# foxcroftjn/polars-strsim

Measured on AMD Instinct MI355X. Metric: M string-pairs/s, levenshtein, 100 M rows (+ achieved HBM GB/s in roofline), higher is better.
Workload: dtype u8/u32 bit-parallel, f64 epilogue

## Files before the change

### polars-strsim_amd/csrc/strsim_capi.cpp

```cpp
#include <hip/hip_runtime.h>
#include <algorithm>

#include <cstdarg>
#include <cstdio>
#include <cstdlib>
#include <cstring>
#include <memory>
#include <new>
#include <string>

#include "strsim_amd.h"
#include "strsim_internal.h"
#include "strsim_kernels.h"
#define STRSIM_OSA_NO_KERNELS
#include "strsim_osa.h"
#include "strsim_distance.h"
#include "strsim_indel.h"
#include "strsim_partial.h"
#include "strsim_token.h"
#include "strsim_nearest.h"

namespace strsim {

static thread_local std::string g_last_error;
// ... 324 lines not shown
    if (const char *env = getenv("STRSIM_LEV_WAVES_PER_CU")) {
        const int v = atoi(env);
        if (v >= 1 && v <= 256) c->lev_waves_per_cu = v;
    }
    c->no_literal_path = getenv("STRSIM_NO_LITERAL_PATH") != nullptr;
    if (const char *env = getenv("STRSIM_WIDE_WG_PER_CU")) {
        const int v = atoi(env);
        if (v >= 1 && v <= 4096) c->wide_cap_per_cu = v;
    }
    if (const char *env = getenv("STRSIM_HUGE_WAVES_PER_CU")) {
        const int v = atoi(env);
        if (v >= 1 && v <= 32) c->huge_waves_per_cu = v;
    }
    if (const char *env = getenv("STRSIM_HOST_DIRECT_ROWS")) c->host_direct_rows = (uint64_t)strtoull(env, nullptr, 10);
    if (const char *env = getenv("STRSIM_FAULT_RETIRE_AT")) c->fault_retire_at = (uint64_t)strtoull(env, nullptr, 10);
    if (hip_stream) {
        c->stream = (hipStream_t)hip_stream;
    } else {
        e = hipStreamCreateWithFlags(&c->stream, hipStreamNonBlocking);
        if (e != hipSuccess) { delete c; return hip_fail(e, "hipStreamCreateWithFlags"); }
        c->own_stream = true;
    }
    e = hipMalloc((void **)&c->status, sizeof(DevStatus) * strsim_ctx::RING);
    if (e == hipSuccess) e = hipMalloc((void **)&c->sched, sizeof(uint32_t) * 4 * strsim_ctx::RING);
    if (e == hipSuccess) e = hipMemsetAsync(c->sched, 0, sizeof(uint32_t) * 4 * strsim_ctx::RING, c->stream);
    if (e == hipSuccess)
        e = hipHostMalloc((void **)&c->status_host, sizeof(DevStatus) * strsim_ctx::RING, hipHostMallocDefault);
    if (e != hipSuccess) { strsim_ctx_destroy(c); return hip_fail(e, "status allocation"); }
    memset(c->status_host, 0, sizeof(DevStatus) * strsim_ctx::RING);
    e = hipHostGetDevicePointer((void **)&c->status_host_dev, c->status_host, 0);
    if (e != hipSuccess) { strsim_ctx_destroy(c); return hip_fail(e, "hipHostGetDevicePointer"); }
    {
        static double q[QTAB_N * QTAB_N];
        for (int a = 0; a < QTAB_N; ++a)
            for (int b = 0; b < QTAB_N; ++b) q[a * QTAB_N + b] = b ? (double)a / (double)b : 0.0;
        e = hipMalloc((void **)&c->qtab, sizeof(q));
        if (e == hipSuccess) e = hipMemcpy(c->qtab, q, sizeof(q), hipMemcpyHostToDevice);
        if (e != hipSuccess) { strsim_ctx_destroy(c); return hip_fail(e, "quotient table"); }
    }
    *out_ctx = c;
    return STRSIM_OK;
}

void strsim_ctx_destroy(strsim_ctx_t *c)
{
    if (!c) return;
    (void)hipSetDevice(c->device);
    if (c->stream) (void)hipStreamSynchronize(c->stream);
// ... 410 lines not shown
    }
    if (two_pass_measure(measure)) return pairs_osa(c, slot, measure, a_off, a_val, a_rows, b_off, b_val, b_rows, outs[0], n);
    if (measure == STRSIM_TOKEN_SORT_RATIO || measure == STRSIM_TOKEN_SET_RATIO)
        return pairs_token(c, slot, measure, a_off, a_val, a_rows, b_off, b_val, b_rows, outs[0], n);
    const uint64_t nchunks = (n + 63) >> 6;
    bool defer = !eager && !c->expect_slow && !c->stream_ordered;
    int mb = strsim_ctx::SHARED_MASKBUF;
    if (defer) {
        defer = false;
        for (int b = 0; b < strsim_ctx::SHARED_MASKBUF; ++b)
            if (c->maskbuf_owner[b] < 0) { mb = b; defer = true; break; }
    }
    rc = c->slowmask[mb].reserve(2 * nchunks * sizeof(unsigned long long) + nchunks * sizeof(uint32_t));
    if (rc) return rc;
    unsigned long long *const mask = c->slowmask[mb].as<unsigned long long>();
    slot_begin(c, slot);
    c->status_host[slot].lane_left = LANE_LEFT_UNKNOWN;

    LaunchArgs la;
    la.offA = a_off; la.valA = a_val; la.rowsA = a_rows;
    la.offB = b_off; la.valB = b_val; la.rowsB = b_rows;
    la.out = outs[0]; la.n = n;
    la.slowmask = mask; la.status = c->status + slot; la.stream = c->stream;
    la.sched = c->sched + 4 * slot;
    la.publish_host = nullptr;
    la.publish_ticket = 0u;
    la.worklist = reinterpret_cast<uint32_t *>(mask + 2 * nchunks);
    la.qtab = c->qtab;
    la.stage_grid = c->num_cu * c->stage_wg_per_cu;
    la.no_literal_path = c->no_literal_path;
    la.long_rows = c->long_rows;
    la.wide_grid = c->num_cu * 3;
    la.wide_grid_cap = c->num_cu * c->wide_cap_per_cu;
    la.wave_grid = c->num_cu * 16;
    la.wave_grid_lev = c->num_cu * c->lev_waves_per_cu;
    {
        const size_t waves = (size_t)std::max(la.wave_grid, la.wave_grid_lev);
        rc = c->lev_ws.reserve(waves * LEV_WS_WORDS * sizeof(uint32_t));
        if (rc) return rc;
        la.lev_ws = c->lev_ws.as<uint32_t>();
    }
    la.ev_lane0 = la.ev_lane1 = la.ev_wave1 = nullptr;
    if (c->timing) {
        for (int i = 0; i < 3; ++i)
            if (!c->ev[slot][i]) HIP_TRY(hipEventCreateWithFlags(&c->ev[slot][i], hipEventDisableSystemFence));
        la.ev_lane0 = c->ev[slot][0]; la.ev_lane1 = c->ev[slot][1]; la.ev_wave1 = c->ev[slot][2];
    }
// ... 657 lines not shown
```

### polars-strsim_amd/csrc/strsim_kernels.h

```cpp
#pragma once
#include <hip/hip_runtime.h>
#include <stdint.h>

#include "strsim_lane_core.h"

namespace strsim {

constexpr int WAVE_CAP = 1024;

#ifndef STRSIM_LEV_JOBS
#define STRSIM_LEV_JOBS 16
#endif
constexpr int LEV_JOBS = STRSIM_LEV_JOBS;
#ifndef STRSIM_LEV_BYTES_ROWS
#define STRSIM_LEV_BYTES_ROWS 64
#endif
constexpr int LEV_BYTES_ROWS = STRSIM_LEV_BYTES_ROWS;
#ifndef STRSIM_LEV_POOL
#define STRSIM_LEV_POOL 384
#endif
constexpr int LEV_POOL = STRSIM_LEV_POOL;
constexpr int TXT_PAD = 48;
constexpr int ARENA0_BYTES = 8192;
constexpr int ARENA1_BYTES = 12288;
constexpr int PAT1_BYTES = 64 * 32 * 2;
constexpr int LEV_WS_WORDS = 3 * (WAVE_CAP + 64) + (ARENA0_BYTES + ARENA1_BYTES + PAT1_BYTES) / 4;

#define HUGE_WS_WORDS(cap) (6u * ((uint64_t)(cap) + 64u) + 64u)

struct DevStatus {
    unsigned int wave_rows;
    unsigned int huge_rows;
    unsigned int max_len;
    unsigned int lane_left;
    unsigned int list_count[5];
    unsigned int list_rows[5];
    unsigned int next_entry[5];
    unsigned int pad1[12];
    unsigned int ticket;
};
static_assert(sizeof(DevStatus) == 128, "DevStatus is 128 bytes");

struct LaunchArgs {
    const uint32_t *offA; const uint8_t *valA; uint64_t rowsA;
    const uint32_t *offB; const uint8_t *valB; uint64_t rowsB;
    double *out; uint64_t n;
    unsigned long long *slowmask;
    uint32_t *worklist;
    const double *qtab;
    DevStatus *status;
    uint32_t *sched;
    DevStatus *publish_host;
    uint32_t publish_ticket;
    hipStream_t stream;
    int wide_grid, wave_grid;
    bool no_literal_path;
    bool long_rows;
    int stage_grid;
    int wide_grid_cap;
    int wave_grid_lev;
    uint32_t *lev_ws;
    hipEvent_t ev_lane0, ev_lane1, ev_wave1;
};

// ... 85 lines not shown
```

### polars-strsim_amd/csrc/strsim_lane_stage.h

```cpp
#pragma once

#ifndef STRSIM_STAGE_ROWS
#define STRSIM_STAGE_ROWS 512
#endif
#ifndef STRSIM_STAGE_CAP
#define STRSIM_STAGE_CAP 10240
#endif
#ifndef STRSIM_STAGE_CAP_LONG
#define STRSIM_STAGE_CAP_LONG 15104
#endif
#ifndef STRSIM_STAGE_CAP_LUT
#define STRSIM_STAGE_CAP_LUT 8960
#endif
#ifndef STRSIM_STAGE_WAVES_PER_EU
#define STRSIM_STAGE_WAVES_PER_EU 5
#endif
#ifndef STRSIM_STAGE_BUCKET_SHIFT
#define STRSIM_STAGE_BUCKET_SHIFT 1
#endif

#ifndef STRSIM_STAGE_LUT
#define STRSIM_STAGE_LUT 0x26
#endif
#ifndef STRSIM_JARO_KEEP_EQ_FILLS
#define STRSIM_JARO_KEEP_EQ_FILLS 1
#endif
#ifndef STRSIM_STAGE_LONG_TEXT_MAX
#define STRSIM_STAGE_LONG_TEXT_MAX 32
#endif
#ifndef STRSIM_STAGE_RANGE_MAX
#define STRSIM_STAGE_RANGE_MAX 64
#endif
#ifndef STRSIM_STAGE_RANGE_DIV
#define STRSIM_STAGE_RANGE_DIV 4
#endif
#ifndef STRSIM_STAGE_RANGE_MIN_BLOCKS
#define STRSIM_STAGE_RANGE_MIN_BLOCKS 2
#endif

#if defined(STRSIM_LAB) && defined(STRSIM_STAGE_STAMPS)
__device__ unsigned long long g_stage_stamps[16384][16];
#define STAGE_STAMP(cat) do { __builtin_amdgcn_sched_barrier(0); const unsigned long long t_ = __builtin_amdgcn_s_memtime(); \
                              __builtin_amdgcn_sched_barrier(0); st_acc[cat] += t_ - st_last; st_last = t_; } while (0)
#else
#define STAGE_STAMP(cat) do { } while (0)
#endif

#ifndef STRSIM_STAGE_THREADS
#define STRSIM_STAGE_THREADS 256
#endif
constexpr int STAGE_BLOCK = STRSIM_STAGE_THREADS;
constexpr int STAGE_WAVES = STAGE_BLOCK / 64;
constexpr int STAGE_ROWS = STRSIM_STAGE_ROWS;
constexpr int STAGE_RPT = STAGE_ROWS / STAGE_BLOCK;
constexpr int STAGE_NR = STAGE_ROWS / 64;
constexpr int STAGE_RPW = STAGE_NR / STAGE_WAVES;
template <int MEASURE> constexpr bool stage_uses_lut() { return ((STRSIM_STAGE_LUT >> MEASURE) & 1) != 0; }

template <bool TABLES, bool LONG = false> struct StageGeom {
    static_assert(!(TABLES && LONG), "the long-row geometry has no match-mask tables");
// ... 228 lines not shown
    constexpr bool LEV = MEASURE == LEVENSHTEIN;
    constexpr bool ALL = MEASURE == ALL_MEASURES;
    constexpr int B = STAGE_ROWS, RPT = STAGE_RPT, NBK = STAGE_NBK;
    constexpr int STAGE_CAP = StageGeom<LUT, LONG>::CAP, STAGE_COL = StageGeom<LUT, LONG>::COL;
    constexpr int STAGE_DMA_ITERS = StageGeom<LUT, LONG>::DMA_ITERS;
    constexpr uint32_t COLB = STAGE_COL, LIT = 2u * STAGE_COL;
    static_assert(!LUT || (B <= 128 * STAGE_WAVES && LUT_WAVE_BYTES == 3072), "descriptor slices: 128 rows behind each wave's tables");
    __shared__ __attribute__((aligned(4096))) uint8_t s_lut[LUT ? 4096 * STAGE_WAVES : 16];
    __shared__ uint2 s_desc_own[LUT ? 1 : B];
    __shared__ __attribute__((aligned(4096))) uint8_t s_bytes[2 * STAGE_COL + 64 + 16];
    auto desc_at = [&](uint32_t p) -> uint2 * {
        if (LUT) return reinterpret_cast<uint2 *>(s_lut + ((p >> 7) << 12) + LUT_WAVE_BYTES + ((p & 127u) << 3));
        return s_desc_own + p;
    };
    __shared__ __attribute__((aligned(16))) uint32_t s_off[2][B + 4];
    __shared__ uint32_t s_cnt[32];
    __shared__ uint32_t s_left;
    __shared__ uint32_t s_sched[2];
    __shared__ uint16_t s_code[LEV ? B : 1];
    __shared__ uint32_t s_word[(!LEV && !ALL) ? B : 1];
    __shared__ double s_val[ALL ? B : 1];

    const uint32_t tid = threadIdx.x, lane = lane_id(), wv = tid >> 6;
    if (blockIdx.x == 0u && tid < (uint32_t)(sizeof(DevStatus) / sizeof(uint32_t))) reinterpret_cast<uint32_t *>(status)[tid] = 0u;
    if (tid < 32u) s_cnt[tid] = 0u;
    if (tid == 0u) s_left = 0u;
#pragma unroll
    for (int q = 0; q < RPT; ++q) {
        const uint32_t i = (uint32_t)q * STAGE_BLOCK + tid;
        if (LEV) s_code[i] = 0xFFFFu;
        else if (ALL) reinterpret_cast<unsigned long long *>(&s_val[i])[0] = ~0ull;
        else s_word[i] = 0xFFFFFFFFu;
    }

    const uint32_t totalA = load_invariant(offA + rowsA), totalB = load_invariant(offB + rowsB);
#if STRSIM_BOUNDS_ON
    const uint32_t firstA = load_invariant(offA), firstB = load_invariant(offB);
#endif
    const bool bcastA = rowsA == 1, bcastB = rowsB == 1;
    const uint32_t litA0 = bcastA ? load_invariant(offA) : 0u, litB0 = bcastB ? load_invariant(offB) : 0u;
    const uint32_t litAlen = bcastA ? totalA - litA0 : 0u, litBlen = bcastB ? totalB - litB0 : 0u;
    if (wv == 0u) {
        auto literal_window = [&](const uint8_t *val, uint32_t at, uint32_t total, uint32_t len, uint32_t *dst) {
            uint32_t w[8];
            load_window32(val, at, total, w);
            const uint32_t rep = (w[0] & 0xFFu) * 0x01010101u;
#pragma unroll
            for (int q = 0; q < 8; ++q) {
                const uint32_t v = len > 4u * q ? (len - 4u * q < 4u ? len - 4u * q : 4u) : 0u;
                const uint32_t keep = v >= 4u ? 0xFFFFFFFFu : ((1u << (8u * v)) - 1u);
                dst[q] = (w[q] & keep) | (rep & ~keep);
            }
        };
        if (bcastA) literal_window(valA, litA0, totalA, litAlen, reinterpret_cast<uint32_t *>(s_bytes + LIT));
        if (bcastB) literal_window(valB, litB0, totalB, litBlen, reinterpret_cast<uint32_t *>(s_bytes + LIT + 32u));
    }
    const uint64_t nchunks = (n + 63u) >> 6;
    const uint32_t nchunks32 = (uint32_t)nchunks;
    auto grab = [&](uint32_t seen, uint32_t &lo, uint32_t &sz) {
        const uint32_t left = nchunks32 > seen ? nchunks32 - seen : 0u;
        uint32_t want = (uint32_t)STRSIM_STAGE_RANGE_MAX;
        if (left < (uint32_t)(STRSIM_STAGE_RANGE_MAX * STRSIM_STAGE_RANGE_DIV) * gridDim.x) want = left / ((uint32_t)STRSIM_STAGE_RANGE_DIV * gridDim.x);
        sz = want < (uint32_t)(STRSIM_STAGE_RANGE_MIN_BLOCKS * (B / 64)) ? (uint32_t)(STRSIM_STAGE_RANGE_MIN_BLOCKS * (B / 64)) : want;
        lo = __hip_atomic_fetch_add(&sched[0], sz, __ATOMIC_RELAXED, __HIP_MEMORY_SCOPE_AGENT);
    };
    uint32_t grab_lo = 0u, grab_sz = 0u;
    if (tid == 0u) {
        grab(0u, grab_lo, grab_sz);
        s_sched[0] = grab_lo;
        s_sched[1] = grab_sz;
    }
    lds_barrier();
    uint64_t row_end;
    uint64_t row0;
    {
        const uint64_t lo = uniform(s_sched[0]), hi = lo + uniform(s_sched[1]);
        row0 = lo * 64u < n ? lo * 64u : n;
        row_end = hi * 64u < n ? hi * 64u : n;
    }
    lds_barrier();
    if (tid == 0u) grab(grab_lo, grab_lo, grab_sz);
    bool grab_pending = true;

    EqLut lut;
    lut.lane4 = lane * 4u;
    lut.krep = ((STRSIM_LDS_ADDR(&s_lut[0]) >> 8) + 16u * wv) * 0x01010101u;
    const uint32_t ldsOffA = STRSIM_LDS_ADDR(&s_off[0][0]), ldsOffB = STRSIM_LDS_ADDR(&s_off[1][0]);
    const uint32_t ldsBytes = STRSIM_LDS_ADDR(&s_bytes[0]);
    const uint32_t wvu = uniform(wv);
    const uint32_t tid4 = tid * 4u, tid16 = tid * 16u;
    auto dma_offsets = [&](uint64_t row) {
        const uint32_t cnt = (uint32_t)(row_end - row < (uint64_t)B ? row_end - row : (uint64_t)B);
        const uint32_t *const pa = offA + row, *const pb = offB + row;
#pragma unroll
        for (int it = 0; it < RPT; ++it) {
            if (tid + (uint32_t)it * STAGE_BLOCK <= cnt) {
                if (!bcastA) STRSIM_CHECK_INDEX(K_STAGE, 1, row, row + (uint64_t)it * STAGE_BLOCK + tid, rowsA + 1u);
                if (!bcastB) STRSIM_CHECK_INDEX(K_STAGE, 2, row, row + (uint64_t)it * STAGE_BLOCK + tid, rowsB + 1u);
                STRSIM_CHECK_INDEX(K_STAGE, 3, row, (uint32_t)it * STAGE_BLOCK + tid, B + 4);
                if (!bcastA) lds_dma_b32(pa + it * STAGE_BLOCK, tid4, ldsOffA + 4u * ((uint32_t)it * STAGE_BLOCK + wvu * 64u));
                if (!bcastB) lds_dma_b32(pb + it * STAGE_BLOCK, tid4, ldsOffB + 4u * ((uint32_t)it * STAGE_BLOCK + wvu * 64u));
            }
        }
        if (tid == 0u && cnt == (uint32_t)B) {
            if (!bcastA) STRSIM_CHECK_INDEX(K_STAGE, 4, row, row + (uint64_t)B, rowsA + 1u);
            if (!bcastB) STRSIM_CHECK_INDEX(K_STAGE, 5, row, row + (uint64_t)B, rowsB + 1u);
            if (!bcastA) lds_dma_b32(pa + B, tid4, ldsOffA + 4u * (uint32_t)B);
            if (!bcastB) lds_dma_b32(pb + B, tid4, ldsOffB + 4u * (uint32_t)B);
        }
    };

    uint64_t prev_row0 = 0;
    uint32_t prev_rows = 0;
    if (row0 < row_end) dma_offsets(row0);
    asm volatile("s_waitcnt vmcnt(0)" ::: "memory");
    lds_barrier();

    auto pin = [](double &x) { asm volatile("" : "+v"(x)); };
    auto store_block = [&](uint64_t r0, uint32_t rows) {
        unsigned long long *__restrict__ const maskb = slowmask + (r0 >> 6);
        constexpr int M1 = (MEASURE == ALL_MEASURES || MEASURE == LEVENSHTEIN) ? JARO : MEASURE;
        constexpr bool JARO_LIKE = ALL || M1 == JARO || M1 == JARO_WINKLER;
        unsigned long long pk[RPT];
        double t0[RPT], t1[RPT], t2[RPT], t3[RPT];
#pragma unroll
        for (int q = 0; q < RPT; ++q) {
            const uint32_t i = (uint32_t)q * STAGE_BLOCK + tid;
            if (ALL) {
                pk[q] = reinterpret_cast<const unsigned long long *>(s_val)[i];
                reinterpret_cast<unsigned long long *>(s_val)[i] = ~0ull;
            } else if (LEV) {
                pk[q] = s_code[i];
                s_code[i] = 0xFFFFu;
            } else {
                pk[q] = s_word[i];
                s_word[i] = 0xFFFFFFFFu;
            }
        }
#pragma unroll
// ... 47 lines not shown
                if (valid && !undone) {
                    if (ALL) {
#pragma unroll
                        for (int o = 0; o < 5; ++o) outs.p[o][r0 + i] = v5[o];
                    } else {
                        outs.p[0][r0 + i] = v;
                    }
                }
                if (lane == 0u && valid) {
                    maskb[i >> 6] = left;
                    if (publish && left) atomicAdd(&s_left, (uint32_t)__builtin_popcountll(left));
                }
            }
        }
    };

#if defined(STRSIM_LAB) && defined(STRSIM_STAGE_STAMPS)
    unsigned long long st_acc[10] = {0, 0, 0, 0, 0, 0, 0, 0, 0, 0};
    const unsigned long long st_t0 = __builtin_amdgcn_s_memtime(), st_r0 = __builtin_amdgcn_s_memrealtime();
    unsigned long long st_last = st_t0;
#endif
    while (row0 < row_end) {
        if (grab_pending) {
            if (tid == 0u) {
                s_sched[0] = grab_lo;
                s_sched[1] = grab_sz;
            }
            grab_pending = false;
        }
        if (prev_rows) store_block(prev_row0, prev_rows);
        STAGE_STAMP(1);
        const uint32_t avail = (uint32_t)(row_end - row0 < (uint64_t)B ? row_end - row0 : (uint64_t)B);
        const uint32_t baseA = bcastA ? litA0 : uniform(s_off[0][0]), baseB = bcastB ? litB0 : uniform(s_off[1][0]);
        const uint32_t misA = (uint32_t)(reinterpret_cast<uintptr_t>(valA + baseA) & 15u);
        const uint32_t misB = (uint32_t)(reinterpret_cast<uintptr_t>(valB + baseB) & 15u);
        uint32_t rows;
        {
            const uint32_t e = (lane + 1u) * 64u < avail ? (lane + 1u) * 64u : avail;
            const bool exists = lane * 64u < avail && lane < (uint32_t)(B / 64);
            const uint32_t endA = bcastA ? baseA : s_off[0][exists ? e : 0u], endB = bcastB ? baseB : s_off[1][exists ? e : 0u];
            const bool fits = exists && endA - baseA + misA <= (uint32_t)STAGE_CAP && endB - baseB + misB <= (uint32_t)STAGE_CAP;
            const unsigned long long okm = __ballot(fits);
            uint32_t k = (uint32_t)__builtin_ctzll(~okm);
            if (k == 0u) k = 1u;
            rows = uniform(k * 64u < avail ? k * 64u : avail);
        }
        const uint32_t endA = bcastA ? baseA : uniform(s_off[0][rows]), endB = bcastB ? baseB : uniform(s_off[1][rows]);
        const uint32_t spanA = endA - baseA + misA, spanB = endB - baseB + misB;
        const uint32_t stagedA = bcastA ? 0u : (((spanA < (uint32_t)STAGE_CAP ? spanA : (uint32_t)STAGE_CAP) + 15u) & ~15u);
        const uint32_t stagedB = bcastB ? 0u : (((spanB < (uint32_t)STAGE_CAP ? spanB : (uint32_t)STAGE_CAP) + 15u) & ~15u);
// ... 68 lines not shown
#pragma unroll
            for (int q = 0; q < RPT; ++q) {
                const uint32_t base = __shfl(exc, skey[q], 32);
                const uint32_t p = base + srank[q];
                STRSIM_CHECK_INDEX(K_STAGE, 31, row0, p, B);
                *desc_at(p) = make_uint2(sd0[q], sd1[q]);
            }
            nmine = uniform(__shfl(exc, NBK - 1, 32));
        }
        STAGE_STAMP(4);
        asm volatile("s_waitcnt vmcnt(0)" ::: "memory");
        if (!bcastA && leftA < (chunksA << 4) && tid == ((chunksA - 1u) & (uint32_t)(STAGE_BLOCK - 1)))
            for (uint32_t b = leftA; b < (chunksA << 4); ++b) { STRSIM_CHECK_INDEX(K_STAGE, 32, row0, b, COLB); s_bytes[b] = 0; }
        if (!bcastB && leftB < (chunksB << 4) && tid == ((chunksB - 1u) & (uint32_t)(STAGE_BLOCK - 1)))
            for (uint32_t b = leftB; b < (chunksB << 4); ++b) { STRSIM_CHECK_INDEX(K_STAGE, 33, row0, COLB + b, sizeof(s_bytes)); s_bytes[COLB + b] = 0; }
        lds_barrier();
        STAGE_STAMP(5);
        if (tid < 32u) s_cnt[tid] = 0u;
        uint64_t next_row0 = row0 + rows;
        if (next_row0 >= row_end) {
            const uint64_t lo = uniform(s_sched[0]), hi = lo + uniform(s_sched[1]);
            next_row0 = lo * 64u < n ? lo * 64u : n;
            row_end = hi * 64u < n ? hi * 64u : n;
            if (tid == 0u) grab((uint32_t)lo, grab_lo, grab_sz);
            grab_pending = true;
        }
        if (next_row0 < row_end) dma_offsets(next_row0);
        STAGE_STAMP(6);
        __builtin_amdgcn_s_setprio(0);
        {
            const uint32_t nrounds = (nmine + 63u) >> 6;
#pragma unroll 1
            for (int k = 0; k < STAGE_RPW; ++k) {
                const uint32_t t = (uint32_t)(k >> 1) * (2u * STAGE_WAVES) + ((k & 1) ? (uint32_t)(2 * STAGE_WAVES - 1) - wv : wv);
                if (t >= nrounds) continue;
                const uint32_t hi = nmine - 64u * t;
                const uint32_t first = hi >= 64u ? hi - 64u : 0u;
                const uint32_t in_round = hi - first;
                __builtin_amdgcn_s_setprio(1);
                STRSIM_CHECK_INDEX(K_STAGE, 41, row0, first + lane, B);
                const uint2 d = *desc_at(first + lane);
                uint32_t wt[8], wp[8];
                stage_window(s_bytes, d.x & 0xFFFFu, wt, (uint32_t)sizeof(s_bytes), STRSIM_BOUNDS_ON ? 1u : 0u);
                stage_window(s_bytes, d.x >> 16, wp, (uint32_t)sizeof(s_bytes), STRSIM_BOUNDS_ON ? 1u : 0u);
    #if defined(STRSIM_LAB) && defined(STRSIM_STAGE_STAMPS)
                asm volatile("s_waitcnt lgkmcnt(0)" ::: "memory");
    #endif
                STAGE_STAMP(7);
                __builtin_amdgcn_s_setprio(0);
                stage_compute<MEASURE, LUT>(lut, wt, wp, lane < in_round ? d.y : STAGE_DEAD, in_round - 1u, s_code, s_word, s_val);
                STAGE_STAMP(8);
            }
        }
        __builtin_amdgcn_s_setprio(1);
        asm volatile("s_waitcnt vmcnt(0)" ::: "memory");
        lds_barrier();
        STAGE_STAMP(9);
        prev_row0 = row0;
        prev_rows = rows;
        row0 = next_row0;
    }
    if (prev_rows) store_block(prev_row0, prev_rows);
    if (publish) lds_barrier();
    if (tid == 0u) {
        if (publish && s_left) __hip_atomic_fetch_add(&sched[2], s_left, __ATOMIC_RELAXED, __HIP_MEMORY_SCOPE_AGENT);
        const uint32_t done = __hip_atomic_fetch_add(&sched[1], 1u, __ATOMIC_ACQ_REL, __HIP_MEMORY_SCOPE_AGENT);
        if (done == gridDim.x - 1u) {
            if (publish) {
                const uint32_t total = __hip_atomic_load(&sched[2], __ATOMIC_RELAXED, __HIP_MEMORY_SCOPE_AGENT);
                __hip_atomic_store(&publish->lane_left, total, __ATOMIC_RELEASE, __HIP_MEMORY_SCOPE_SYSTEM);
                if (ticket) __hip_atomic_store(&publish->ticket, ticket, __ATOMIC_RELEASE, __HIP_MEMORY_SCOPE_SYSTEM);
            }
            __hip_atomic_store(&sched[0], 0u, __ATOMIC_RELAXED, __HIP_MEMORY_SCOPE_AGENT);
            __hip_atomic_store(&sched[1], 0u, __ATOMIC_RELAXED, __HIP_MEMORY_SCOPE_AGENT);
            __hip_atomic_store(&sched[2], 0u, __ATOMIC_RELAXED, __HIP_MEMORY_SCOPE_AGENT);
        }
    }
#if defined(STRSIM_LAB) && defined(STRSIM_STAGE_STAMPS)
    if (lane == 0u) {
        const uint32_t w = (blockIdx.x * STAGE_WAVES + wv) & 16383u;
        for (int q = 0; q < 10; ++q) g_stage_stamps[w][q] = st_acc[q];
        g_stage_stamps[w][10] = __builtin_amdgcn_s_memtime() - st_t0;
        const unsigned long long st_r1 = __builtin_amdgcn_s_memrealtime();
        g_stage_stamps[w][11] = st_r1 - st_r0;
        g_stage_stamps[w][12] = st_r0;
        g_stage_stamps[w][13] = st_r1;
        g_stage_stamps[w][14] = (unsigned long long)__builtin_amdgcn_s_getreg((4 << 0) | (0 << 6) | (31 << 11));
        g_stage_stamps[w][15] = (unsigned long long)__builtin_amdgcn_s_getreg((20 << 0) | (0 << 6) | (31 << 11));
    }
#endif
}

#ifndef STRSIM_STAGE_PLAIN_WAVES
#define STRSIM_STAGE_PLAIN_WAVES 5
#endif
#ifndef STRSIM_STAGE_ALL_WAVES_PER_EU
#define STRSIM_STAGE_ALL_WAVES_PER_EU 3
#endif
template <int MEASURE, bool TABLES, bool LONG = false> constexpr int stage_waves_per_eu()
{
    constexpr int lim = MEASURE == ALL_MEASURES ? STRSIM_STAGE_ALL_WAVES_PER_EU : ((TABLES || LONG) ? 4 : STRSIM_STAGE_PLAIN_WAVES);
    return STRSIM_STAGE_WAVES_PER_EU < lim ? STRSIM_STAGE_WAVES_PER_EU : lim;
}

template <int MEASURE, bool TABLES, bool LONG = false>
__global__ __launch_bounds__(STAGE_BLOCK) __attribute__((amdgpu_waves_per_eu(stage_waves_per_eu<MEASURE, TABLES, LONG>()))) void
k_lane_stage(const uint32_t *__restrict__ offA, const uint8_t *__restrict__ valA, uint64_t rowsA,
             const uint32_t *__restrict__ offB, const uint8_t *__restrict__ valB, uint64_t rowsB, OutPtrs outs, uint64_t n,
             unsigned long long *__restrict__ slowmask, DevStatus *__restrict__ status, const double *__restrict__ qtab,
             uint32_t *__restrict__ sched, DevStatus *__restrict__ publish, uint32_t ticket)
{
// ... 12 lines not shown
```

Measured before the change: 70180.

## Shard stage work-stealing counter and optionally seed static first ranges

Replaces the single global atomic chunk counter in the stage kernel with a sharded set of counters on separate cache lines. Each workgroup draws from its home shard and steals from the fullest shard when its own is exhausted. An optional mode hands every workgroup a static first range before it touches any dynamic counter. The first range's offset DMA is now issued before the literal-window setup, and a microbenchmark for same-address atomic contention plus a stamp-analysis script are added. With the default settings (one shard, no static first) the behaviour is close to the old single counter, with somewhat more bookkeeping per draw.

```diff
diff --git a/bench_support/micro/atomic_same_address.hip b/bench_support/micro/atomic_same_address.hip
--- /dev/null
+++ b/bench_support/micro/atomic_same_address.hip
@@ -0,0 +1,66 @@
+#include <hip/hip_runtime.h>
+#include <cstdio>
+#include <cstdint>
+#include <cstdlib>
+#include <algorithm>
+#include <vector>
+
+#define CHECK(x) do { hipError_t e_ = (x); if (e_ != hipSuccess) { printf("%s: %s\n", #x, hipGetErrorString(e_)); return 1; } } while (0)
+
+__global__ __launch_bounds__(256) void k(uint32_t *counters, int shards, int iters, unsigned long long *stamps, uint32_t *sink)
+{
+    if (threadIdx.x != 0) return;
+    uint32_t *c = counters + 32 * (blockIdx.x % (unsigned)shards);
+    const unsigned long long r0 = __builtin_amdgcn_s_memrealtime();
+    uint32_t acc = __hip_atomic_fetch_add(c, 1u, __ATOMIC_RELAXED, __HIP_MEMORY_SCOPE_AGENT);
+    asm volatile("s_waitcnt vmcnt(0)" : "+v"(acc) : : "memory");
+    const unsigned long long r1 = __builtin_amdgcn_s_memrealtime();
+#pragma unroll 1
+    for (int i = 1; i < iters; ++i) {
+        acc += __hip_atomic_fetch_add(c, 1u + (acc & 1u), __ATOMIC_RELAXED, __HIP_MEMORY_SCOPE_AGENT);
+    }
+    asm volatile("s_waitcnt vmcnt(0)" : "+v"(acc) : : "memory");
+    const unsigned long long r2 = __builtin_amdgcn_s_memrealtime();
+    stamps[3 * blockIdx.x + 0] = r0;
+    stamps[3 * blockIdx.x + 1] = r1;
+    stamps[3 * blockIdx.x + 2] = r2;
+    sink[blockIdx.x] = acc;
+}
+
+int main(int argc, char **argv)
+{
+    const int grid = argc > 1 ? atoi(argv[1]) : 1280, iters = argc > 2 ? atoi(argv[2]) : 200;
+    uint32_t *counters, *sink;
+    unsigned long long *stamps;
+    CHECK(hipMalloc((void **)&counters, 64 * 128));
+    CHECK(hipMalloc((void **)&sink, grid * sizeof(uint32_t)));
+    CHECK(hipMalloc((void **)&stamps, 3 * grid * sizeof(unsigned long long)));
+    std::vector<unsigned long long> h(3 * (size_t)grid);
+    printf("grid %d workgroups, %d dependent fetch_add per workgroup (thread 0), s_memrealtime at 100 MHz\n", grid, iters);
+    const int shard_counts[] = {1, 2, 8, 32, 64};
+    for (int s : shard_counts) {
+        for (int rep = 0; rep < 3; ++rep) {
+            CHECK(hipMemset(counters, 0, 64 * 128));
+            hipLaunchKernelGGL(k, dim3(grid), dim3(256), 0, 0, counters, s, iters, stamps, sink);
+            CHECK(hipDeviceSynchronize());
+        }
+        CHECK(hipMemcpy(h.data(), stamps, h.size() * sizeof(unsigned long long), hipMemcpyDeviceToHost));
+        unsigned long long first = ~0ull, last = 0, last_first_result = 0;
+        std::vector<double> lat1, latn;
+        for (int b = 0; b < grid; ++b) {
+            first = std::min(first, h[3 * b]);
+            last = std::max(last, h[3 * b + 2]);
+            last_first_result = std::max(last_first_result, h[3 * b + 1]);
+            lat1.push_back((double)(h[3 * b + 1] - h[3 * b]) * 10.0);
+            latn.push_back((double)(h[3 * b + 2] - h[3 * b + 1]) * 10.0 / (double)std::max(iters - 1, 1));
+        }
+        std::sort(lat1.begin(), lat1.end());
+        std::sort(latn.begin(), latn.end());
+        const double total_ns = (double)(last - first) * 10.0, n = (double)grid * iters;
+        printf("S = %2d: %8.1f us for %8.0f atomics = %6.1f ns each overall (%5.1f ns per atomic and address); first result of a workgroup "
+               "p50 %6.0f ns max %6.0f ns, the last workgroup has it %6.1f us after the first entry; later ones p50 %6.0f ns p99 %6.0f ns\n",
+               s, total_ns / 1e3, n, total_ns / n, total_ns / n * s, lat1[lat1.size() / 2], lat1.back(), (double)(last_first_result - first) / 100.0,
+               latn[latn.size() / 2], latn[(latn.size() * 99) / 100]);
+    }
+    return 0;
+}
diff --git a/bench_support/stage_launch_stamps.py b/bench_support/stage_launch_stamps.py
--- /dev/null
+++ b/bench_support/stage_launch_stamps.py
@@ -0,0 +1,76 @@
+import ctypes as C
+import os
+import sys
+import time
+
+import numpy as np
+
+ROOT = os.path.dirname(os.path.dirname(os.path.abspath(__file__)))
+sys.path.insert(0, os.path.join(ROOT, "polars-strsim_amd"))
+sys.path.insert(0, ROOT)
+import torch
+import strsim_amd as S
+from bench_support import workload as W
+
+rows = int(sys.argv[1]) if len(sys.argv) > 1 else 12_500_000
+mode = sys.argv[2] if len(sys.argv) > 2 else "one_launch"
+reads = int(sys.argv[3]) if len(sys.argv) > 3 else 3
+assert mode in ("one_launch", "stream_ordered")
+dev = torch.device("cuda", 0)
+measure, _, law, lo, hi, seed = W.CONFIGS["cfg2"]
+oa, va, ob, vb, _, _ = W.device_columns(seed, law, lo, hi, 0, rows, dev)
+out = torch.empty(rows, dtype=torch.float64, device=dev)
+st = torch.cuda.Stream()
+torch.cuda.set_stream(st)
+ctx = S.Context(0, stream=st.cuda_stream, one_launch=(mode == "one_launch"))
+f = S.lib().strsim_debug_stage_stamps
+f.argtypes = [C.c_void_p, C.c_size_t]
+f.restype = C.c_int
+NW = 16384
+
+
+def pct(x):
+    return "min %7.1f  p10 %7.1f  p50 %7.1f  p90 %7.1f  p99 %7.1f  max %7.1f" % (x.min(), np.percentile(x, 10), np.median(x), np.percentile(x, 90),
+                                                                            np.percentile(x, 99), x.max())
+
+
+print("cfg2 %s, %d rows, %s calls, library %s" % (measure, rows, mode, os.path.basename(os.environ.get("STRSIM_AMD_LIB", "(in tree)"))))
+for _ in range(20):
+    ctx.pairs_device(measure, oa, va, ob, vb, out=out)
+ctx.synchronize()
+t0 = time.perf_counter()
+for _ in range(20):
+    ctx.pairs_device(measure, oa, va, ob, vb, out=out)
+ctx.synchronize()
+print("wall clock per call, 20 calls back to back: %.1f us" % ((time.perf_counter() - t0) / 20 * 1e6))
+for r in range(reads):
+    ops0 = ctx.enqueued_ops
+    ctx.pairs_device(measure, oa, va, ob, vb, out=out)
+    ctx.synchronize()
+    torch.cuda.synchronize()
+    buf = np.zeros((NW, 16), dtype=np.uint64)
+    assert f(buf.ctypes.data, NW) == 0
+    used = buf[:, 13] > 0
+    nw = int(np.nonzero(used)[0].max()) + 1 if used.any() else 0
+    nw -= nw % 4
+    b = buf[:nw].astype(np.float64)
+    wg = nw // 4
+    t_first = b[:, 12].min()
+    entry = ((b[:, 12] - t_first) / 100.0).reshape(wg, 4).min(axis=1)
+    rounds = np.where(buf[:nw, 14] > 0, (b[:, 14] - t_first) / 100.0, np.nan).reshape(wg, 4)
+    has_rounds = ~np.isnan(rounds).all(axis=1)
+    first_rounds = np.nanmin(rounds[has_rounds], axis=1)
+    end = ((b[:, 13] - t_first) / 100.0).reshape(wg, 4).max(axis=1)
+    ghz = b[:, 10].sum() / max(b[:, 11].sum(), 1.0) * 0.1
+    w0 = buf[:nw:4, 15]
+    draws = ((w0 >> np.uint64(4)) & np.uint64(0xFFF)).astype(np.float64)
+    wait_us = (w0 >> np.uint64(16)).astype(np.float64) / (ghz * 1e3)
+    print("launch %d: %d operations enqueued, %d workgroups (%d with rounds), kernel %.1f us, clock of the stamps %.2f GHz" %
+          (r, ctx.enqueued_ops - ops0, wg, int(has_rounds.sum()), end.max(), ghz))
+    print("  workgroup entry - first entry, us:        " + pct(entry))
+    print("  first rounds - first entry, us:           " + pct(first_rounds))
+    print("  first rounds - own entry, us:             " + pct(first_rounds - entry[has_rounds]))
+    print("  workgroup end - first entry, us:          " + pct(end))
+    print("  last end - workgroup end (idle tail), us: " + pct(end.max() - end) + "   mean %.1f" % (end.max() - end).mean())
+    print("  draws per workgroup:                      " + pct(draws) + "   total %d" % int(draws.sum()))
+    print("  wait for draws per workgroup, us:         " + pct(wait_us) + "   per draw %.2f us" % (wait_us.sum() / max(draws.sum(), 1.0)))
diff --git a/polars-strsim_amd/csrc/strsim_capi.cpp b/polars-strsim_amd/csrc/strsim_capi.cpp
--- a/polars-strsim_amd/csrc/strsim_capi.cpp
+++ b/polars-strsim_amd/csrc/strsim_capi.cpp
@@ -370,8 +370,8 @@
         c->own_stream = true;
     }
     e = hipMalloc((void **)&c->status, sizeof(DevStatus) * strsim_ctx::RING);
-    if (e == hipSuccess) e = hipMalloc((void **)&c->sched, sizeof(uint32_t) * 4 * strsim_ctx::RING);
-    if (e == hipSuccess) e = hipMemsetAsync(c->sched, 0, sizeof(uint32_t) * 4 * strsim_ctx::RING, c->stream);
+    if (e == hipSuccess) e = hipMalloc((void **)&c->sched, sizeof(uint32_t) * strsim::SCHED_SLOT_WORDS * strsim_ctx::RING);
+    if (e == hipSuccess) e = hipMemsetAsync(c->sched, 0, sizeof(uint32_t) * strsim::SCHED_SLOT_WORDS * strsim_ctx::RING, c->stream);
     if (e == hipSuccess)
         e = hipHostMalloc((void **)&c->status_host, sizeof(DevStatus) * strsim_ctx::RING, hipHostMallocDefault);
     if (e != hipSuccess) { strsim_ctx_destroy(c); return hip_fail(e, "status allocation"); }
@@ -828,7 +828,7 @@
     la.offB = b_off; la.valB = b_val; la.rowsB = b_rows;
     la.out = outs[0]; la.n = n;
     la.slowmask = mask; la.status = c->status + slot; la.stream = c->stream;
-    la.sched = c->sched + 4 * slot;
+    la.sched = c->sched + strsim::SCHED_SLOT_WORDS * slot;
     la.publish_host = nullptr;
     la.publish_ticket = 0u;
     la.worklist = reinterpret_cast<uint32_t *>(mask + 2 * nchunks);
diff --git a/polars-strsim_amd/csrc/strsim_kernels.h b/polars-strsim_amd/csrc/strsim_kernels.h
--- a/polars-strsim_amd/csrc/strsim_kernels.h
+++ b/polars-strsim_amd/csrc/strsim_kernels.h
@@ -40,6 +40,105 @@
     unsigned int ticket;
 };
 static_assert(sizeof(DevStatus) == 128, "DevStatus is 128 bytes");
+
+#ifndef STRSIM_STAGE_RANGE_MAX
+#define STRSIM_STAGE_RANGE_MAX 64
+#endif
+#ifndef STRSIM_STAGE_RANGE_DIV
+#define STRSIM_STAGE_RANGE_DIV 4
+#endif
+#ifndef STRSIM_STAGE_RANGE_MIN_BLOCKS
+#define STRSIM_STAGE_RANGE_MIN_BLOCKS 2
+#endif
+#ifndef STRSIM_STAGE_SHARDS
+#define STRSIM_STAGE_SHARDS 1
+#endif
+#ifndef STRSIM_STAGE_STATIC_FIRST
+#define STRSIM_STAGE_STATIC_FIRST 0
+#endif
+#ifndef STRSIM_STAGE_ROWS
+#define STRSIM_STAGE_ROWS 512
+#endif
+constexpr int STAGE_SHARDS = STRSIM_STAGE_SHARDS;
+constexpr int SCHED_LINE_WORDS = 32;
+constexpr int SCHED_SLOT_WORDS = (1 + STAGE_SHARDS) * SCHED_LINE_WORDS;
+constexpr uint32_t STAGE_RANGE_MIN_CHUNKS = (uint32_t)(STRSIM_STAGE_RANGE_MIN_BLOCKS * (STRSIM_STAGE_ROWS / 64));
+static_assert(STAGE_SHARDS >= 1 && STAGE_SHARDS <= 64 && (STAGE_SHARDS & (STAGE_SHARDS - 1)) == 0, "STRSIM_STAGE_SHARDS: a power of two, at most 64");
+static_assert(STRSIM_STAGE_RANGE_MAX >= 1 && STRSIM_STAGE_RANGE_MAX <= 255 && STAGE_RANGE_MIN_CHUNKS <= 255u, "a range's size travels in eight bits");
+
+STRSIM_HD uint32_t stage_range_size(uint32_t left, uint32_t grid)
+{
+    uint32_t want = (uint32_t)STRSIM_STAGE_RANGE_MAX;
+    static_assert(STRSIM_STAGE_RANGE_DIV >= 1 && (uint64_t)STRSIM_STAGE_RANGE_MAX * STRSIM_STAGE_RANGE_DIV <= 4095u, "RANGE_MAX x RANGE_DIV x 2^20 fits 32 bits");
+    const uint32_t per = (uint32_t)STRSIM_STAGE_RANGE_DIV * (grid == 0u ? 1u : (grid < (1u << 20) ? grid : (1u << 20)));
+    if (left < (uint32_t)STRSIM_STAGE_RANGE_MAX * per) want = left / per;
+    return want < STAGE_RANGE_MIN_CHUNKS ? STAGE_RANGE_MIN_CHUNKS : want;
+}
+
+struct StageSplit {
+    uint32_t first;
+    uint32_t static_end;
+    uint32_t slice;
+};
+
+STRSIM_HD StageSplit stage_split(uint32_t nchunks, uint32_t grid)
+{
+    StageSplit sp;
+    sp.first = STRSIM_STAGE_STATIC_FIRST ? stage_range_size(nchunks, grid) : 0u;
+    const uint64_t se = (uint64_t)sp.first * (uint64_t)grid;
+    sp.static_end = se < (uint64_t)nchunks ? (uint32_t)se : nchunks;
+    sp.slice = (uint32_t)(((uint64_t)(nchunks - sp.static_end) + (uint64_t)(STAGE_SHARDS - 1)) / (uint64_t)STAGE_SHARDS);
+    return sp;
+}
+
+STRSIM_HD void stage_static_range(const StageSplit &sp, uint32_t nchunks, uint32_t b, uint32_t &lo, uint32_t &cnt)
+{
+    const uint64_t l = (uint64_t)b * (uint64_t)sp.first;
+    if (l >= (uint64_t)sp.static_end) { lo = nchunks; cnt = 0u; return; }
+    lo = (uint32_t)l;
+    cnt = sp.static_end - lo < sp.first ? sp.static_end - lo : sp.first;
+}
+
+STRSIM_HD uint32_t stage_shard_len(const StageSplit &sp, uint32_t nchunks, uint32_t s)
+{
+    const uint64_t at = (uint64_t)s * (uint64_t)sp.slice, rem = (uint64_t)(nchunks - sp.static_end);
+    if (at >= rem) return 0u;
+    return rem - at < (uint64_t)sp.slice ? (uint32_t)(rem - at) : sp.slice;
+}
+
+STRSIM_HD uint32_t stage_draw_size(const StageSplit &sp, uint32_t nchunks, uint32_t grid, uint32_t s, uint32_t seen)
+{
+    const uint32_t len = stage_shard_len(sp, nchunks, s);
+    const uint64_t left = (uint64_t)(len > seen ? len - seen : 0u) * (uint64_t)STAGE_SHARDS;
+    return stage_range_size(left > 0xFFFFFFFFull ? 0xFFFFFFFFu : (uint32_t)left, grid);
+}
+
+STRSIM_HD bool stage_draw_range(const StageSplit &sp, uint32_t nchunks, uint32_t s, uint32_t got, uint32_t sz, uint32_t &lo, uint32_t &cnt)
+{
+    const uint32_t len = stage_shard_len(sp, nchunks, s);
+    if (got >= len) { lo = nchunks; cnt = 0u; return false; }
+    lo = sp.static_end + s * sp.slice + got;
+    cnt = len - got < sz ? len - got : sz;
+    return true;
+}
+
+STRSIM_HD int stage_pick_shard(const StageSplit &sp, uint32_t nchunks, uint32_t grid, const uint32_t (&seen)[STAGE_SHARDS], uint32_t &sz)
+{
+    int pick = -1;
+    uint32_t best = 0u;
+    uint64_t total = 0u;
+#if defined(__HIPCC__)
+#pragma unroll
+#endif
+    for (int s = 0; s < STAGE_SHARDS; ++s) {
+        const uint32_t len = stage_shard_len(sp, nchunks, (uint32_t)s);
+        const uint32_t left = len > seen[s] ? len - seen[s] : 0u;
+        total += left;
+        if (left > best) { best = left; pick = s; }
+    }
+    sz = stage_range_size(total > 0xFFFFFFFFull ? 0xFFFFFFFFu : (uint32_t)total, grid);
+    return pick;
+}
 
 struct LaunchArgs {
     const uint32_t *offA; const uint8_t *valA; uint64_t rowsA;
diff --git a/polars-strsim_amd/csrc/strsim_lane_stage.h b/polars-strsim_amd/csrc/strsim_lane_stage.h
--- a/polars-strsim_amd/csrc/strsim_lane_stage.h
+++ b/polars-strsim_amd/csrc/strsim_lane_stage.h
@@ -27,15 +27,6 @@
 #endif
 #ifndef STRSIM_STAGE_LONG_TEXT_MAX
 #define STRSIM_STAGE_LONG_TEXT_MAX 32
-#endif
-#ifndef STRSIM_STAGE_RANGE_MAX
-#define STRSIM_STAGE_RANGE_MAX 64
-#endif
-#ifndef STRSIM_STAGE_RANGE_DIV
-#define STRSIM_STAGE_RANGE_DIV 4
-#endif
-#ifndef STRSIM_STAGE_RANGE_MIN_BLOCKS
-#define STRSIM_STAGE_RANGE_MIN_BLOCKS 2
 #endif
 
 #if defined(STRSIM_LAB) && defined(STRSIM_STAGE_STAMPS)
@@ -310,6 +301,103 @@
     __shared__ double s_val[ALL ? B : 1];
 
     const uint32_t tid = threadIdx.x, lane = lane_id(), wv = tid >> 6;
+#if defined(STRSIM_LAB) && defined(STRSIM_STAGE_STAMPS)
+    const unsigned long long st_entry = __builtin_amdgcn_s_memrealtime();
+    unsigned long long st_grab = 0, st_first = 0;
+#endif
+    const uint64_t nchunks = (n + 63u) >> 6;
+    const uint32_t nchunks32 = (uint32_t)nchunks;
+    const StageSplit split = stage_split(nchunks32, gridDim.x);
+    const bool dynamic = split.static_end < nchunks32;
+    auto counter = [&](uint32_t shard) -> uint32_t * {
+        STRSIM_CHECK_INDEX(K_STAGE, 50, ~0ull, (1u + shard) * (uint32_t)SCHED_LINE_WORDS, SCHED_SLOT_WORDS);
+        return sched + (1u + shard) * (uint32_t)SCHED_LINE_WORDS;
+    };
+    uint32_t grab_got = 0u, grab_req = 0u;
+    auto grab = [&](uint32_t shard, uint32_t seen) {
+        const uint32_t sz = stage_draw_size(split, nchunks32, gridDim.x, shard, seen);
+        grab_req = (shard << 8) | sz;
+#if defined(STRSIM_LAB) && defined(STRSIM_STAGE_STAMPS)
+        const unsigned long long g0 = __builtin_amdgcn_s_memtime();
+#endif
+        grab_got = __hip_atomic_fetch_add(counter(shard), sz, __ATOMIC_RELAXED, __HIP_MEMORY_SCOPE_AGENT);
+#if defined(STRSIM_LAB) && defined(STRSIM_STAGE_STAMPS)
+        asm volatile("s_waitcnt vmcnt(0)" : "+v"(grab_got) : : "memory");
+        st_grab += (__builtin_amdgcn_s_memtime() - g0) + (1ull << 48);
+#endif
+    };
+    auto publish_grab = [&]() {
+        uint32_t lo, cnt;
+        uint32_t shard = grab_req >> 8;
+        if (!stage_draw_range(split, nchunks32, shard, grab_got, grab_req & 0xFFu, lo, cnt) && STAGE_SHARDS > 1) {
+            for (;;) {
+                uint32_t seen[STAGE_SHARDS];
+#pragma unroll
+                for (int q = 0; q < STAGE_SHARDS; ++q) seen[q] = __hip_atomic_load(counter((uint32_t)q), __ATOMIC_RELAXED, __HIP_MEMORY_SCOPE_AGENT);
+                uint32_t sz;
+                const int pick = stage_pick_shard(split, nchunks32, gridDim.x, seen, sz);
+                if (pick < 0) break;
+                shard = (uint32_t)pick;
+                const uint32_t got = __hip_atomic_fetch_add(counter(shard), sz, __ATOMIC_RELAXED, __HIP_MEMORY_SCOPE_AGENT);
+                grab_got = got;
+                grab_req = (shard << 8) | sz;
+                if (stage_draw_range(split, nchunks32, shard, got, sz, lo, cnt)) break;
+            }
+        }
+        s_sched[0] = lo;
+        s_sched[1] = cnt;
+    };
+    uint64_t row_end;
+    uint64_t row0;
+    bool grab_pending = false;
+    bool first_grab = false;
+    const uint32_t home = blockIdx.x & (uint32_t)(STAGE_SHARDS - 1);
+
+    const bool bcastA = rowsA == 1, bcastB = rowsB == 1;
+    const uint32_t ldsOffA = STRSIM_LDS_ADDR(&s_off[0][0]), ldsOffB = STRSIM_LDS_ADDR(&s_off[1][0]);
+    const uint32_t ldsBytes = STRSIM_LDS_ADDR(&s_bytes[0]);
+    const uint32_t wvu = uniform(wv);
+    const uint32_t tid4 = tid * 4u, tid16 = tid * 16u;
+    auto dma_offsets = [&](uint64_t row_) {
+        const uint64_t row = ((uint64_t)uniform((uint32_t)(row_ >> 32)) << 32) | (uint64_t)uniform((uint32_t)row_);
+        const uint32_t cnt = (uint32_t)(row_end - row < (uint64_t)B ? row_end - row : (uint64_t)B);
+        const uint32_t *const pa = offA + row, *const pb = offB + row;
+#pragma unroll
+        for (int it = 0; it < RPT; ++it) {
+            if (tid + (uint32_t)it * STAGE_BLOCK <= cnt) {
+                if (!bcastA) STRSIM_CHECK_INDEX(K_STAGE, 1, row, row + (uint64_t)it * STAGE_BLOCK + tid, rowsA + 1u);
+                if (!bcastB) STRSIM_CHECK_INDEX(K_STAGE, 2, row, row + (uint64_t)it * STAGE_BLOCK + tid, rowsB + 1u);
+                STRSIM_CHECK_INDEX(K_STAGE, 3, row, (uint32_t)it * STAGE_BLOCK + tid, B + 4);
+                if (!bcastA) lds_dma_b32(pa + it * STAGE_BLOCK, tid4, ldsOffA + 4u * ((uint32_t)it * STAGE_BLOCK + wvu * 64u));
+                if (!bcastB) lds_dma_b32(pb + it * STAGE_BLOCK, tid4, ldsOffB + 4u * ((uint32_t)it * STAGE_BLOCK + wvu * 64u));
+            }
+        }
+        if (tid == 0u && cnt == (uint32_t)B) {
+            if (!bcastA) STRSIM_CHECK_INDEX(K_STAGE, 4, row, row + (uint64_t)B, rowsA + 1u);
+            if (!bcastB) STRSIM_CHECK_INDEX(K_STAGE, 5, row, row + (uint64_t)B, rowsB + 1u);
+            if (!bcastA) lds_dma_b32(pa + B, tid4, ldsOffA + 4u * (uint32_t)B);
+            if (!bcastB) lds_dma_b32(pb + B, tid4, ldsOffB + 4u * (uint32_t)B);
+        }
+    };
+
+#if STRSIM_STAGE_STATIC_FIRST
+    {
+        uint32_t lo32, cnt32;
+        stage_static_range(split, nchunks32, blockIdx.x, lo32, cnt32);
+        const uint64_t lo = uniform(lo32), hi = lo + uniform(cnt32);
+        row0 = lo * 64u < n ? lo * 64u : n;
+        row_end = hi * 64u < n ? hi * 64u : n;
+        if (row0 < row_end) dma_offsets(row0);
+        if (tid == 0u) {
+            s_sched[0] = nchunks32;
+            s_sched[1] = 0u;
+        }
+        if (dynamic) {
+            if (row_end - row0 > (uint64_t)B) first_grab = true;
+            else grab_pending = true;
+        }
+    }
+#endif
     if (blockIdx.x == 0u && tid < (uint32_t)(sizeof(DevStatus) / sizeof(uint32_t))) reinterpret_cast<uint32_t *>(status)[tid] = 0u;
     if (tid < 32u) s_cnt[tid] = 0u;
     if (tid == 0u) s_left = 0u;
@@ -325,7 +413,6 @@
 #if STRSIM_BOUNDS_ON
     const uint32_t firstA = load_invariant(offA), firstB = load_invariant(offB);
 #endif
-    const bool bcastA = rowsA == 1, bcastB = rowsB == 1;
     const uint32_t litA0 = bcastA ? load_invariant(offA) : 0u, litB0 = bcastB ? load_invariant(offB) : 0u;
     const uint32_t litAlen = bcastA ? totalA - litA0 : 0u, litBlen = bcastB ? totalB - litB0 : 0u;
     if (wv == 0u) {
@@ -343,66 +430,36 @@
         if (bcastA) literal_window(valA, litA0, totalA, litAlen, reinterpret_cast<uint32_t *>(s_bytes + LIT));
         if (bcastB) literal_window(valB, litB0, totalB, litBlen, reinterpret_cast<uint32_t *>(s_bytes + LIT + 32u));
     }
-    const uint64_t nchunks = (n + 63u) >> 6;
-    const uint32_t nchunks32 = (uint32_t)nchunks;
-    auto grab = [&](uint32_t seen, uint32_t &lo, uint32_t &sz) {
-        const uint32_t left = nchunks32 > seen ? nchunks32 - seen : 0u;
-        uint32_t want = (uint32_t)STRSIM_STAGE_RANGE_MAX;
-        if (left < (uint32_t)(STRSIM_STAGE_RANGE_MAX * STRSIM_STAGE_RANGE_DIV) * gridDim.x) want = left / ((uint32_t)STRSIM_STAGE_RANGE_DIV * gridDim.x);
-        sz = want < (uint32_t)(STRSIM_STAGE_RANGE_MIN_BLOCKS * (B / 64)) ? (uint32_t)(STRSIM_STAGE_RANGE_MIN_BLOCKS * (B / 64)) : want;
-        lo = __hip_atomic_fetch_add(&sched[0], sz, __ATOMIC_RELAXED, __HIP_MEMORY_SCOPE_AGENT);
-    };
-    uint32_t grab_lo = 0u, grab_sz = 0u;
+#if !STRSIM_STAGE_STATIC_FIRST
     if (tid == 0u) {
-        grab(0u, grab_lo, grab_sz);
-        s_sched[0] = grab_lo;
-        s_sched[1] = grab_sz;
+        grab(home, 0u);
+        publish_grab();
     }
     lds_barrier();
-    uint64_t row_end;
-    uint64_t row0;
     {
         const uint64_t lo = uniform(s_sched[0]), hi = lo + uniform(s_sched[1]);
         row0 = lo * 64u < n ? lo * 64u : n;
         row_end = hi * 64u < n ? hi * 64u : n;
     }
     lds_barrier();
-    if (tid == 0u) grab(grab_lo, grab_lo, grab_sz);
-    bool grab_pending = true;
+    if (row0 < row_end) {
+        if (tid == 0u) grab(grab_req >> 8, grab_got);
+        grab_pending = true;
+        dma_offsets(row0);
+    }
+#endif
 
     EqLut lut;
     lut.lane4 = lane * 4u;
     lut.krep = ((STRSIM_LDS_ADDR(&s_lut[0]) >> 8) + 16u * wv) * 0x01010101u;
-    const uint32_t ldsOffA = STRSIM_LDS_ADDR(&s_off[0][0]), ldsOffB = STRSIM_LDS_ADDR(&s_off[1][0]);
-    const uint32_t ldsBytes = STRSIM_LDS_ADDR(&s_bytes[0]);
-    const uint32_t wvu = uniform(wv);
-    const uint32_t tid4 = tid * 4u, tid16 = tid * 16u;
-    auto dma_offsets = [&](uint64_t row) {
-        const uint32_t cnt = (uint32_t)(row_end - row < (uint64_t)B ? row_end - row : (uint64_t)B);
-        const uint32_t *const pa = offA + row, *const pb = offB + row;
-#pragma unroll
-        for (int it = 0; it < RPT; ++it) {
-            if (tid + (uint32_t)it * STAGE_BLOCK <= cnt) {
-                if (!bcastA) STRSIM_CHECK_INDEX(K_STAGE, 1, row, row + (uint64_t)it * STAGE_BLOCK + tid, rowsA + 1u);
-                if (!bcastB) STRSIM_CHECK_INDEX(K_STAGE, 2, row, row + (uint64_t)it * STAGE_BLOCK + tid, rowsB + 1u);
-                STRSIM_CHECK_INDEX(K_STAGE, 3, row, (uint32_t)it * STAGE_BLOCK + tid, B + 4);
-                if (!bcastA) lds_dma_b32(pa + it * STAGE_BLOCK, tid4, ldsOffA + 4u * ((uint32_t)it * STAGE_BLOCK + wvu * 64u));
-                if (!bcastB) lds_dma_b32(pb + it * STAGE_BLOCK, tid4, ldsOffB + 4u * ((uint32_t)it * STAGE_BLOCK + wvu * 64u));
-            }
-        }
-        if (tid == 0u && cnt == (uint32_t)B) {
-            if (!bcastA) STRSIM_CHECK_INDEX(K_STAGE, 4, row, row + (uint64_t)B, rowsA + 1u);
-            if (!bcastB) STRSIM_CHECK_INDEX(K_STAGE, 5, row, row + (uint64_t)B, rowsB + 1u);
-            if (!bcastA) lds_dma_b32(pa + B, tid4, ldsOffA + 4u * (uint32_t)B);
-            if (!bcastB) lds_dma_b32(pb + B, tid4, ldsOffB + 4u * (uint32_t)B);
-        }
-    };
 
     uint64_t prev_row0 = 0;
     uint32_t prev_rows = 0;
-    if (row0 < row_end) dma_offsets(row0);
     asm volatile("s_waitcnt vmcnt(0)" ::: "memory");
     lds_barrier();
+#if STRSIM_STAGE_STATIC_FIRST
+    if (grab_pending && tid == 0u) grab(home, 0u);
+#endif
 
     auto pin = [](double &x) { asm volatile("" : "+v"(x)); };
     auto store_block = [&](uint64_t r0, uint32_t rows) {
@@ -496,10 +553,7 @@
 #endif
     while (row0 < row_end) {
         if (grab_pending) {
-            if (tid == 0u) {
-                s_sched[0] = grab_lo;
-                s_sched[1] = grab_sz;
-            }
+            if (tid == 0u) publish_grab();
             grab_pending = false;
         }
         if (prev_rows) store_block(prev_row0, prev_rows);
@@ -614,11 +668,20 @@
             const uint64_t lo = uniform(s_sched[0]), hi = lo + uniform(s_sched[1]);
             next_row0 = lo * 64u < n ? lo * 64u : n;
             row_end = hi * 64u < n ? hi * 64u : n;
-            if (tid == 0u) grab((uint32_t)lo, grab_lo, grab_sz);
+            if (hi > lo) {
+                if (tid == 0u) grab(grab_req >> 8, grab_got);
+                grab_pending = true;
+            }
+        } else if (first_grab) {
+            if (tid == 0u) grab(home, 0u);
             grab_pending = true;
         }
+        first_grab = false;
         if (next_row0 < row_end) dma_offsets(next_row0);
         STAGE_STAMP(6);
+#if defined(STRSIM_LAB) && defined(STRSIM_STAGE_STAMPS)
+        if (st_first == 0ull) st_first = __builtin_amdgcn_s_memrealtime();
+#endif
         __builtin_amdgcn_s_setprio(0);
         {
             const uint32_t nrounds = (nmine + 63u) >> 6;
@@ -663,9 +726,10 @@
                 __hip_atomic_store(&publish->lane_left, total, __ATOMIC_RELEASE, __HIP_MEMORY_SCOPE_SYSTEM);
                 if (ticket) __hip_atomic_store(&publish->ticket, ticket, __ATOMIC_RELEASE, __HIP_MEMORY_SCOPE_SYSTEM);
             }
-            __hip_atomic_store(&sched[0], 0u, __ATOMIC_RELAXED, __HIP_MEMORY_SCOPE_AGENT);
             __hip_atomic_store(&sched[1], 0u, __ATOMIC_RELAXED, __HIP_MEMORY_SCOPE_AGENT);
             __hip_atomic_store(&sched[2], 0u, __ATOMIC_RELAXED, __HIP_MEMORY_SCOPE_AGENT);
+            if (dynamic)
+                for (uint32_t q = 0; q < (uint32_t)STAGE_SHARDS; ++q) __hip_atomic_store(counter(q), 0u, __ATOMIC_RELAXED, __HIP_MEMORY_SCOPE_AGENT);
         }
     }
 #if defined(STRSIM_LAB) && defined(STRSIM_STAGE_STAMPS)
@@ -675,10 +739,11 @@
         g_stage_stamps[w][10] = __builtin_amdgcn_s_memtime() - st_t0;
         const unsigned long long st_r1 = __builtin_amdgcn_s_memrealtime();
         g_stage_stamps[w][11] = st_r1 - st_r0;
-        g_stage_stamps[w][12] = st_r0;
+        g_stage_stamps[w][12] = st_entry;
         g_stage_stamps[w][13] = st_r1;
-        g_stage_stamps[w][14] = (unsigned long long)__builtin_amdgcn_s_getreg((4 << 0) | (0 << 6) | (31 << 11));
-        g_stage_stamps[w][15] = (unsigned long long)__builtin_amdgcn_s_getreg((20 << 0) | (0 << 6) | (31 << 11));
+        g_stage_stamps[w][14] = st_first;
+        g_stage_stamps[w][15] = ((unsigned long long)__builtin_amdgcn_s_getreg((20 << 0) | (0 << 6) | (31 << 11)) & 15ull)
+                                | ((st_grab >> 48) << 4) | ((st_grab & 0xFFFFFFFFFFFFull) << 16);
     }
 #endif
 }
```

New measurement: 70270, median of 2. About the same (+0.1%).
